# facebookresearch/rela

Measured on AMD Instinct MI355X. Metric: env-steps/s (Ape-X Atari 84x84x4, actor tick + learner grad-step), higher is better.
Workload: dtype f32 (f32 operands as 3 exact bf16 parts on bf16 MFMA; f32-accurate); 1 GPU; Ape-X DQN 80x80 envs/GPU, actor+learner on one MI355X, replay 2^20, B=512, A=18, n=3; device-resident static frames; parallelism=single

## Files before the change

rela_amd/csrc/conv12_s3.h:

```cpp
#pragma once
#include <hip/hip_runtime.h>

#include "gemm_s3.h"

namespace rela_amd {
namespace s3 {

typedef int i32x4 __attribute__((ext_vector_type(4)));
typedef uint32_t u32x4_a4 __attribute__((ext_vector_type(4), aligned(4)));
#ifndef C12_ABLATE
#define C12_ABLATE 0
#endif

constexpr bool kNoCopyOut = C12_ABLATE == 1, kNoStage = C12_ABLATE == 2, kNoEpi1 = C12_ABLATE == 3, kNoEpi2 = C12_ABLATE == 4,
               kNoConv1 = C12_ABLATE == 5, kNoConv2 = C12_ABLATE == 6;

struct Conv12S {
  static constexpr int kT = 256;
  static constexpr int GW = 21, NPIX = GW * GW, PLANE_ELEMS = 84 * 84, IN_ELEMS = 4 * PLANE_ELEMS;
  static constexpr int PLANE1 = 7168;
  static constexpr int T1_BYTES = 4 * PLANE1;
  static constexpr int Q = 13, RQ = 261;
  static constexpr int T2_BYTES = 20 * RQ * 16;
  static constexpr int OROW = 400;
  static constexpr int O_BYTES = 81 * OROW;
  static constexpr int SPARE = T1_BYTES + T2_BYTES + O_BYTES;
  static constexpr int LDS_TOTAL = SPARE + 256;
  static_assert(LDS_TOTAL <= 160 * 1024, "LDS budget");
  static constexpr int OV16 = 81 * 24, OIT = (OV16 + kT - 1) / kT;
  static constexpr int UNITS = 4 * GW * 6, UIT = (UNITS + kT - 1) / kT;
  static constexpr int KS2 = 16;
  static constexpr int tap2(int ks) {
    const int c = ks >> 2, j = ks & 3;
    const int dh = j >> 1, dw = (j ^ (j >> 1)) & 1;
    return (((c >> 1) + 2 * dh) << 2) | ((c & 1) + 2 * dw);
  }
  static constexpr int koff2(int ks) { return ((tap2(ks) >> 2) * RQ + (tap2(ks) & 3) * Q) * 16; }
};

template <bool A1OUT>
__global__ __launch_bounds__(256, 1) void conv12_s3(const uint8_t* __restrict__ in, const uint4* __restrict__ W1d,
                                                    const float* __restrict__ scale1, const float* __restrict__ bias1q,
                                                    const uint4* __restrict__ B2, const float* __restrict__ bias2,
                                                    uint8_t* __restrict__ out, float* __restrict__ a1_out, int N) {
  using F = Conv12S;
  extern __shared__ __attribute__((aligned(16))) uint8_t smem_c12[];
  uint8_t* t1 = smem_c12;
  uint8_t* t2 = t1 + F::T1_BYTES;
  uint8_t* otile = t2 + F::T2_BYTES;
  const int tid = threadIdx.x, lane = tid & 63, li = lane & 15, g = lane >> 4;
  const int wave = __builtin_amdgcn_readfirstlane(tid >> 6);
  const int bid = blockIdx.x, nblk = gridDim.x;
  int n = bid;
  if (n >= N) return;

  const int ct1 = wave & 1, rg1 = wave >> 1;
  bf16x8 w2[F::KS2][3];
  {
    const uint4* bp = B2 + (size_t)wave * 3 * 64 + lane;
#pragma unroll
    for (int ks = 0; ks < F::KS2; ++ks)
#pragma unroll
      for (int p = 0; p < 3; ++p) w2[ks][p] = __builtin_bit_cast(bf16x8, bp[(size_t)(ks * TN * 3 + p) * 64]);
  }
  i32x4 wd[4][3];
#pragma unroll
  for (int ks = 0; ks < 4; ++ks)
#pragma unroll
    for (int d = 0; d < 3; ++d) wd[ks][d] = __builtin_bit_cast(i32x4, W1d[((d * 2 + ct1) * 4 + ks) * 64 + lane]);
  auto pin_weights = [&]() __attribute__((always_inline)) {
#pragma unroll
    for (int ks = 0; ks < F::KS2; ++ks)
#pragma unroll
      for (int p = 0; p < 3; ++p) asm volatile("" : "+a"(w2[ks][p]));
#pragma unroll
    for (int ks = 0; ks < 4; ++ks)
#pragma unroll
      for (int d = 0; d < 3; ++d) asm volatile("" : "+v"(wd[ks][d]));
  };
  pin_weights();
  const int ch1 = ct1 * 16 + 4 * g, ch2 = wave * 16 + 4 * g;
  const f32x4 sc1 = *reinterpret_cast<const f32x4*>(scale1 + ch1), bv1 = *reinterpret_cast<const f32x4*>(bias1q + ch1);
  const f32x4 bv2 = *reinterpret_cast<const f32x4*>(bias2 + ch2);

  u32x4_a4 sq[F::UIT][4];
  uint32_t ugoff[F::UIT], uloff[F::UIT];
#pragma unroll
  for (int j = 0; j < F::UIT; ++j) {
    const int u = min(tid + j * F::kT, F::UNITS - 1);
    const int pl = u / (F::GW * 6), rem = u - pl * (F::GW * 6);
    const int Y = rem / 6, qi = rem - Y * 6;
    const int X0 = qi < 5 ? 4 * qi : 17;
    ugoff[j] = (uint32_t)(pl * F::PLANE_ELEMS + 4 * Y * 84 + 4 * X0);
    uloff[j] = (uint32_t)(pl * F::PLANE1 + (Y * F::GW + X0) * 16);
  }
  auto g_load4 = [&](int fr, int j) __attribute__((always_inline)) {
    const uint8_t* fb = in + (size_t)fr * F::IN_ELEMS;
#pragma unroll
    for (int r = 0; r < 4; ++r) sq[j][r] = *reinterpret_cast<const u32x4_a4*>(fb + (size_t)ugoff[j] + r * 84);
  };
  auto s_store4 = [&](int j, int k) __attribute__((always_inline)) {
    *reinterpret_cast<uint4*>(t1 + uloff[j] + k * 16) = make_uint4(sq[j][0][k] ^ 0x80808080u, sq[j][1][k] ^ 0x80808080u,
                                                                   sq[j][2][k] ^ 0x80808080u, sq[j][3][k] ^ 0x80808080u);
  };

  int prev = -1;
  static_assert(F::OIT == 8, "eight named chunk registers (an array indexed inside the hooks stays in scratch)");
  uint4 oc0, oc1, oc2, oc3, oc4, oc5, oc6, oc7;
  auto oc_at = [&](auto jt) -> uint4& {
    constexpr int j = decltype(jt)::value;
    if constexpr (j == 0) return oc0;
    else if constexpr (j == 1) return oc1;
    else if constexpr (j == 2) return oc2;
    else if constexpr (j == 3) return oc3;
    else if constexpr (j == 4) return oc4;
    else if constexpr (j == 5) return oc5;
    else if constexpr (j == 6) return oc6;
    else return oc7;
  };
  uint32_t oloff[F::OIT];
#pragma unroll
  for (int j = 0; j < F::OIT; ++j) {
    const int i = min(tid + j * F::kT, F::OV16 - 1);
    const int px = i / 24, u = i - px * 24;
    oloff[j] = (uint32_t)(px * F::OROW + u * 16);
  }
  auto o_read = [&](auto jt) __attribute__((always_inline)) {
    constexpr int j = decltype(jt)::value;
    oc_at(jt) = *reinterpret_cast<const uint4*>(otile + oloff[j]);
  };
  auto o_write = [&](auto jt) __attribute__((always_inline)) {
    constexpr int j = decltype(jt)::value;
    const int i = min(tid + j * F::kT, F::OV16 - 1);
    uint8_t* ob = out + (size_t)(prev >= 0 ? prev : n) * (81 * 384);
    *reinterpret_cast<uint4*>(ob + (size_t)(uint32_t)(i * 16)) = oc_at(jt);
  };
  uint32_t c1src[13], c1dst[13];
#pragma unroll
  for (int t = 0; t < 13; ++t) {
    const int rt = min(rg1 + 2 * t, 24);
    const int m = rt * 16 + li;
    const int oy = m / 20, ox = m - oy * 20;
    c1src[t] = (uint32_t)(g * F::PLANE1 + (oy * F::GW + ox) * 16);
    c1dst[t] = (uint32_t)((oy * F::RQ + ox * F::Q) * 16 + ch1 * 2);
  }
  const uint32_t a1lane = (uint32_t)((li * 32 + ch1) * 4);

  auto conv1_pass = [&](auto t0_tag, auto nt_tag, auto&& hook) {
    constexpr int T0 = decltype(t0_tag)::value, NT = decltype(nt_tag)::value;
    i32x4 s_hi[NT], s_mid[NT], s_lo[NT];
    int a1base[NT];
#pragma unroll
    for (int t = 0; t < NT; ++t) {
      s_hi[t] = s_mid[t] = s_lo[t] = i32x4{0, 0, 0, 0};
      a1base[t] = (int)c1src[T0 + t];
    }
    constexpr int TOT = 4 * NT, D = 4;
    uint4 x[D];
    auto a_issue = [&](auto idx_tag, int slot) {
      constexpr int IDX = decltype(idx_tag)::value, KS = IDX / NT, T = IDX - KS * NT;
      x[slot] = *reinterpret_cast<const uint4*>(t1 + a1base[T] + ((KS >> 1) * F::GW + (KS & 1)) * 16);
    };
    static_for<D>([&](auto i) { a_issue(i, decltype(i)::value); });
    __builtin_amdgcn_sched_barrier(0);
    static_for<TOT>([&](auto it) {
      constexpr int IDX = decltype(it)::value, KS = IDX / NT, T = IDX - KS * NT, SLOT = IDX % D;
      const i32x4 xv = __builtin_bit_cast(i32x4, x[SLOT]);
      if constexpr (!kNoConv1) {
        s_hi[T] = __builtin_amdgcn_mfma_i32_16x16x64_i8(wd[KS][0], xv, s_hi[T], 0, 0, 0);
        s_mid[T] = __builtin_amdgcn_mfma_i32_16x16x64_i8(wd[KS][1], xv, s_mid[T], 0, 0, 0);
        s_lo[T] = __builtin_amdgcn_mfma_i32_16x16x64_i8(wd[KS][2], xv, s_lo[T], 0, 0, 0);
      } else {
        asm volatile("" ::"v"(xv));
      }
      if constexpr (IDX + D < TOT) a_issue(IC<IDX + D>{}, SLOT);
      hook(IC<T0 * 4 + IDX>{});
      __builtin_amdgcn_sched_barrier(0);
    });
#pragma unroll
    for (int t = 0; t < NT; ++t) asm volatile("" : "+a"(s_hi[t]), "+a"(s_mid[t]), "+a"(s_lo[t]));
#pragma unroll
    for (int t = 0; t < (kNoEpi1 ? 0 : NT); ++t) {
      const int rt = min(rg1 + 2 * (T0 + t), 24);
      const i32x4 ml = s_mid[t] * 256 + s_lo[t];
      const f32x4 hf = __builtin_convertvector(s_hi[t], f32x4), lf = __builtin_convertvector(ml, f32x4);
      f32x4 v;
#pragma unroll
      for (int r = 0; r < 4; ++r) {
        const float u = __builtin_fmaf(hf[r], 65536.0f, lf[r]);
        const float y = __builtin_fmaf(u, sc1[r], bv1[r]);
        v[r] = y > 0.f ? y : 0.f;
      }
      uint2 p0, p1, p2;
      split3_4(v, p0, p1, p2);
      uint8_t* rec = t2 + c1dst[T0 + t];
      *reinterpret_cast<uint2*>(rec) = p0;
      *reinterpret_cast<uint2*>(rec + 64) = p1;
      *reinterpret_cast<uint2*>(rec + 128) = p2;
      if constexpr (A1OUT) {
        uint8_t* ab = reinterpret_cast<uint8_t*>(a1_out + ((size_t)n * 400 + rt * 16) * 32);
        *reinterpret_cast<f32x4*>(ab + (size_t)a1lane) = v;
      }
    }
  };

#pragma unroll
  for (int j = 0; j < F::UIT; ++j) g_load4(n, j);
#pragma unroll
  for (int j = 0; j < F::UIT; ++j)
#pragma unroll
    for (int k = 0; k < 4; ++k) s_store4(j, k);
  __syncthreads();

  auto copy_hook = [&](auto idx_tag) {
    constexpr int IDX = decltype(idx_tag)::value;
    if constexpr (!kNoCopyOut && IDX < 2 * F::OIT) {
      if constexpr (IDX % 2 == 0) o_read(IC<IDX / 2>{});
      else o_write(IC<IDX / 2>{});
    }
  };
  auto no_hook = [](auto) {};
  static_assert(2 * F::OIT <= 20, "copy-out slots inside conv1's first pass");

  uint32_t xbh[6];
#pragma unroll
  for (int t = 0; t < 6; ++t) {
    const int m = t * 16 + li, mm = m < 81 ? m : 80;
    const int oy = mm / 9, ox = mm - oy * 9;
    xbh[t] = (uint32_t)((2 * oy * F::RQ + 2 * ox * F::Q + g) * 16);
  }
  uint32_t o2dst[6];
#pragma unroll
  for (int t = 0; t < 6; ++t) {
    const int m = t * 16 + li;
    o2dst[t] = (uint32_t)((m < 81 ? F::T1_BYTES + F::T2_BYTES + m * F::OROW : F::SPARE) + ch2 * 2);
  }
  for (; n < N; n += nblk) {
    const int nn = (n + nblk < N) ? n + nblk : n;
    pin_weights();
    conv1_pass(IC<0>{}, IC<5>{}, copy_hook);
    conv1_pass(IC<5>{}, IC<4>{}, no_hook);
    conv1_pass(IC<9>{}, IC<4>{}, no_hook);
    if constexpr (kNoEpi1) asm volatile("" ::"v"(sc1), "v"(bv1));
    __syncthreads();
    {
      constexpr int NTILE = 6, TOT = NTILE * F::KS2, D = 3;
      static_assert(NTILE == 6, "xbh / o2dst");
      uint4 xr[D][3];
      auto a_issue = [&](auto idx_tag, int slot) {
        constexpr int IDX = decltype(idx_tag)::value, T = IDX / F::KS2, KS = IDX - T * F::KS2;
        const uint8_t* ap = t2 + xbh[T] + F::koff2(KS);
        xr[slot][0] = *reinterpret_cast<const uint4*>(ap);
        xr[slot][1] = *reinterpret_cast<const uint4*>(ap + 64);
        xr[slot][2] = *reinterpret_cast<const uint4*>(ap + 128);
      };
      static_for<D>([&](auto i) { a_issue(i, decltype(i)::value); });
      __builtin_amdgcn_sched_barrier(0);
      f32x4 acc = bv2, accs = {0.f, 0.f, 0.f, 0.f};
      static_for<TOT>([&](auto it) {
        constexpr int IDX = decltype(it)::value, T = IDX / F::KS2, KS = IDX - T * F::KS2, SLOT = IDX % D;
        const bf16x8 x0 = __builtin_bit_cast(bf16x8, xr[SLOT][0]), x1 = __builtin_bit_cast(bf16x8, xr[SLOT][1]),
                     x2 = __builtin_bit_cast(bf16x8, xr[SLOT][2]);
        if constexpr (!kNoConv2) {
          accs = __builtin_amdgcn_mfma_f32_16x16x32_bf16(w2[KS][2], x0, accs, 0, 0, 0);
          accs = __builtin_amdgcn_mfma_f32_16x16x32_bf16(w2[KS][0], x2, accs, 0, 0, 0);
          accs = __builtin_amdgcn_mfma_f32_16x16x32_bf16(w2[KS][1], x1, accs, 0, 0, 0);
          accs = __builtin_amdgcn_mfma_f32_16x16x32_bf16(w2[KS][1], x0, accs, 0, 0, 0);
          accs = __builtin_amdgcn_mfma_f32_16x16x32_bf16(w2[KS][0], x1, accs, 0, 0, 0);
          acc = __builtin_amdgcn_mfma_f32_16x16x32_bf16(w2[KS][0], x0, acc, 0, 0, 0);
        } else {
          asm volatile("" ::"v"(x0), "v"(x1), "v"(x2));
        }
        if constexpr (IDX + D < TOT) a_issue(IC<IDX + D>{}, SLOT);
        static_for<4 * F::UIT>([&](auto jj) {
          constexpr int JJ = decltype(jj)::value;
          if constexpr (JJ < F::UIT && IDX == 1 + 12 * JJ && !kNoStage) g_load4(nn, JJ);
          if constexpr (IDX == TOT / 2 + 4 * JJ && !kNoStage) s_store4(JJ >> 2, JJ & 3);
        });
        if constexpr (KS == F::KS2 - 1 && kNoEpi2) asm volatile("" ::"v"(acc), "v"(accs));
        if constexpr (KS == F::KS2 - 1 && !kNoEpi2) {
          f32x4 v = acc + accs;
#pragma unroll
          for (int r = 0; r < 4; ++r) v[r] = v[r] > 0.f ? v[r] : 0.f;
          uint2 p0, p1, p2;
          split3_4(v, p0, p1, p2);
          uint8_t* rec = smem_c12 + o2dst[T];
          *reinterpret_cast<uint2*>(rec) = p0;
          *reinterpret_cast<uint2*>(rec + 128) = p1;
          *reinterpret_cast<uint2*>(rec + 256) = p2;
          acc = bv2, accs = f32x4{0.f, 0.f, 0.f, 0.f};
        }
        __builtin_amdgcn_sched_barrier(0);
      });
    }
    __syncthreads();
    prev = n;
  }
  {
    uint4* dst = reinterpret_cast<uint4*>(out + (size_t)prev * (81 * 384));
    for (int i = tid; i < F::OV16; i += F::kT) {
      const int px = i / 24, u = i - px * 24;
      dst[i] = *reinterpret_cast<const uint4*>(otile + px * F::OROW + u * 16);
    }
  }
}

}
}
```

Before: 3.436 million env-steps/s.

## Batch conv2's ragged 81st pixel across images in an LDS ring

Conv2 previously ran six 16-pixel MFMA tiles per image, and the sixth tile carried only one valid pixel (pixel 80). The change runs five full tiles per image and copies pixel 80's input patch into an LDS ring slot. Once five images have accumulated, or the loop ends, it computes one tile whose lanes correspond to different images and writes results straight to global memory. This removes roughly a sixth of conv2's MFMA work, at the cost of extra LDS, a batched tail tile, and scattered global stores that bypass the staged copy-out.

```diff
diff --git a/rela_amd/csrc/conv12_s3.h b/rela_amd/csrc/conv12_s3.h
--- a/rela_amd/csrc/conv12_s3.h
+++ b/rela_amd/csrc/conv12_s3.h
@@ -23,11 +23,15 @@
   static constexpr int Q = 13, RQ = 261;
   static constexpr int T2_BYTES = 20 * RQ * 16;
   static constexpr int OROW = 400;
-  static constexpr int O_BYTES = 81 * OROW;
-  static constexpr int SPARE = T1_BYTES + T2_BYTES + O_BYTES;
-  static constexpr int LDS_TOTAL = SPARE + 256;
+  static constexpr int C2TILES = 5, C2PIX = C2TILES * 16;
+  static constexpr int O_BYTES = C2PIX * OROW;
+  static constexpr int RING_S = 5;
+  static constexpr int PATCH_UNITS = 16 * 12, SLOT_BYTES = 202 * 16;
+  static constexpr int RING = T1_BYTES + T2_BYTES + O_BYTES;
+  static constexpr int LDS_TOTAL = RING + RING_S * SLOT_BYTES;
   static_assert(LDS_TOTAL <= 160 * 1024, "LDS budget");
-  static constexpr int OV16 = 81 * 24, OIT = (OV16 + kT - 1) / kT;
+  static_assert(RING_S >= 1 && RING_S <= 16, "one slot per lane of a tile's column");
+  static constexpr int OV16 = C2PIX * 24, OIT = (OV16 + kT - 1) / kT;
   static constexpr int UNITS = 4 * GW * 6, UIT = (UNITS + kT - 1) / kT;
   static constexpr int KS2 = 16;
   static constexpr int tap2(int ks) {
@@ -222,19 +226,70 @@
   auto no_hook = [](auto) {};
   static_assert(2 * F::OIT <= 20, "copy-out slots inside conv1's first pass");
 
-  uint32_t xbh[6];
-#pragma unroll
-  for (int t = 0; t < 6; ++t) {
-    const int m = t * 16 + li, mm = m < 81 ? m : 80;
-    const int oy = mm / 9, ox = mm - oy * 9;
+  uint32_t xbh[F::C2TILES];
+#pragma unroll
+  for (int t = 0; t < F::C2TILES; ++t) {
+    const int m = t * 16 + li;
+    const int oy = m / 9, ox = m - oy * 9;
     xbh[t] = (uint32_t)((2 * oy * F::RQ + 2 * ox * F::Q + g) * 16);
   }
-  uint32_t o2dst[6];
-#pragma unroll
-  for (int t = 0; t < 6; ++t) {
-    const int m = t * 16 + li;
-    o2dst[t] = (uint32_t)((m < 81 ? F::T1_BYTES + F::T2_BYTES + m * F::OROW : F::SPARE) + ch2 * 2);
-  }
+  uint32_t o2dst[F::C2TILES];
+#pragma unroll
+  for (int t = 0; t < F::C2TILES; ++t) o2dst[t] = (uint32_t)(F::T1_BYTES + F::T2_BYTES + (t * 16 + li) * F::OROW + ch2 * 2);
+  uint32_t psrc, pdst;
+  {
+    const int t = min(tid, F::PATCH_UNITS - 1);
+    const int r = t / 12, u = t - r * 12;
+    psrc = (uint32_t)(((16 + (r >> 2)) * F::RQ + (16 + (r & 3)) * F::Q + u) * 16);
+    pdst = (uint32_t)(F::RING + t * 16);
+  }
+  auto pixel80_tile = [&](int cnt, int first) {
+    constexpr int D = 3;
+    const int sl = min(li, cnt - 1);
+    const uint8_t* rp = smem_c12 + F::RING + sl * F::SLOT_BYTES + g * 16;
+    uint4 xr[D][3];
+    auto a_issue = [&](auto ks_tag, int slot) {
+      constexpr int KS = decltype(ks_tag)::value;
+      const uint8_t* ap = rp + F::tap2(KS) * 192;
+      xr[slot][0] = *reinterpret_cast<const uint4*>(ap);
+      xr[slot][1] = *reinterpret_cast<const uint4*>(ap + 64);
+      xr[slot][2] = *reinterpret_cast<const uint4*>(ap + 128);
+    };
+    static_for<D>([&](auto i) { a_issue(i, decltype(i)::value); });
+    __builtin_amdgcn_sched_barrier(0);
+    f32x4 acc = bv2, accs = {0.f, 0.f, 0.f, 0.f};
+    static_for<F::KS2>([&](auto it) {
+      constexpr int KS = decltype(it)::value, SLOT = KS % D;
+      const bf16x8 x0 = __builtin_bit_cast(bf16x8, xr[SLOT][0]), x1 = __builtin_bit_cast(bf16x8, xr[SLOT][1]),
+                   x2 = __builtin_bit_cast(bf16x8, xr[SLOT][2]);
+      if constexpr (!kNoConv2) {
+        accs = __builtin_amdgcn_mfma_f32_16x16x32_bf16(w2[KS][2], x0, accs, 0, 0, 0);
+        accs = __builtin_amdgcn_mfma_f32_16x16x32_bf16(w2[KS][0], x2, accs, 0, 0, 0);
+        accs = __builtin_amdgcn_mfma_f32_16x16x32_bf16(w2[KS][1], x1, accs, 0, 0, 0);
+        accs = __builtin_amdgcn_mfma_f32_16x16x32_bf16(w2[KS][1], x0, accs, 0, 0, 0);
+        accs = __builtin_amdgcn_mfma_f32_16x16x32_bf16(w2[KS][0], x1, accs, 0, 0, 0);
+        acc = __builtin_amdgcn_mfma_f32_16x16x32_bf16(w2[KS][0], x0, acc, 0, 0, 0);
+      } else {
+        asm volatile("" ::"v"(x0), "v"(x1), "v"(x2));
+      }
+      if constexpr (KS + D < F::KS2) a_issue(IC<KS + D>{}, SLOT);
+      __builtin_amdgcn_sched_barrier(0);
+    });
+    if constexpr (kNoEpi2) {
+      asm volatile("" ::"v"(acc), "v"(accs));
+    } else {
+      f32x4 v = acc + accs;
+#pragma unroll
+      for (int r = 0; r < 4; ++r) v[r] = v[r] > 0.f ? v[r] : 0.f;
+      uint2 p0, p1, p2;
+      split3_4(v, p0, p1, p2);
+      uint8_t* rec = out + (size_t)(first + sl * nblk) * (81 * 384) + (F::C2PIX * 384 + ch2 * 2);
+      *reinterpret_cast<uint2*>(rec) = p0;
+      *reinterpret_cast<uint2*>(rec + 128) = p1;
+      *reinterpret_cast<uint2*>(rec + 256) = p2;
+    }
+  };
+  int filled = 0;
   for (; n < N; n += nblk) {
     const int nn = (n + nblk < N) ? n + nblk : n;
     pin_weights();
@@ -244,8 +299,8 @@
     if constexpr (kNoEpi1) asm volatile("" ::"v"(sc1), "v"(bv1));
     __syncthreads();
     {
-      constexpr int NTILE = 6, TOT = NTILE * F::KS2, D = 3;
-      static_assert(NTILE == 6, "xbh / o2dst");
+      constexpr int TOT = F::C2TILES * F::KS2, D = 3;
+      const uint4 patch = *reinterpret_cast<const uint4*>(t2 + psrc);
       uint4 xr[D][3];
       auto a_issue = [&](auto idx_tag, int slot) {
         constexpr int IDX = decltype(idx_tag)::value, T = IDX / F::KS2, KS = IDX - T * F::KS2;
@@ -272,6 +327,7 @@
           asm volatile("" ::"v"(x0), "v"(x1), "v"(x2));
         }
         if constexpr (IDX + D < TOT) a_issue(IC<IDX + D>{}, SLOT);
+        if constexpr (IDX == 2) *reinterpret_cast<uint4*>(smem_c12 + pdst + filled * F::SLOT_BYTES) = patch;
         static_for<4 * F::UIT>([&](auto jj) {
           constexpr int JJ = decltype(jj)::value;
           if constexpr (JJ < F::UIT && IDX == 1 + 12 * JJ && !kNoStage) g_load4(nn, JJ);
@@ -295,6 +351,10 @@
     }
     __syncthreads();
     prev = n;
+    if (++filled == F::RING_S || n + nblk >= N) {
+      pixel80_tile(filled, n - (filled - 1) * nblk);
+      filled = 0;
+    }
   }
   {
     uint4* dst = reinterpret_cast<uint4*>(out + (size_t)prev * (81 * 384));
```

After: 3.512 million env-steps/s, median of 6. +2.2%, better.
